# thallolang/thallo

Hardware: AMD Instinct MI355X
Metric: pcg_iters_per_sec (higher is better)
Workload: dtype f32

## Files before the change

thallo_amd/csrc/energy_image_warping_march_rc.hip:

```cpp
#include "iw_march.hpp"
#include <hip/hip_ext.h>

using namespace thallo;

namespace {

inline int check_launch() { hipError_t e = hipGetLastError(); return e == hipSuccess ? 0 : -(int)e; }

typedef __amdgpu_buffer_rsrc_t rsrc_t;
typedef unsigned u32x4 __attribute__((ext_vector_type(4)));
typedef unsigned u32x2 __attribute__((ext_vector_type(2)));
__device__ __forceinline__ rsrc_t make_rsrc(const void* p) { return __builtin_amdgcn_make_buffer_rsrc(const_cast<void*>(p), 0, 0xffffffffu, 0x00020000); }
template <bool NT> __device__ __forceinline__ u32x4 bld4(rsrc_t r, unsigned vo, unsigned so) { return __builtin_amdgcn_raw_buffer_load_b128(r, vo, so, NT ? 2 : 0); }
template <bool NT> __device__ __forceinline__ u32x2 bld2(rsrc_t r, unsigned vo, unsigned so) { return __builtin_amdgcn_raw_buffer_load_b64(r, vo, so, NT ? 2 : 0); }
template <bool NT> __device__ __forceinline__ unsigned bld1(rsrc_t r, unsigned vo, unsigned so) { return __builtin_amdgcn_raw_buffer_load_b32(r, vo, so, NT ? 2 : 0); }
template <bool NT> __device__ __forceinline__ void bst4(rsrc_t r, unsigned vo, unsigned so, float a, float b, float c, float d)
{ u32x4 v; v.x = __float_as_uint(a); v.y = __float_as_uint(b); v.z = __float_as_uint(c); v.w = __float_as_uint(d); __builtin_amdgcn_raw_buffer_store_b128(v, r, vo, so, NT ? 2 : 0); }
template <bool NT> __device__ __forceinline__ void bst2(rsrc_t r, unsigned vo, unsigned so, float a, float b)
{ u32x2 v; v.x = __float_as_uint(a); v.y = __float_as_uint(b); __builtin_amdgcn_raw_buffer_store_b64(v, r, vo, so, NT ? 2 : 0); }
__device__ __forceinline__ float uf(unsigned u) { return __uint_as_float(u); }
__device__ __forceinline__ float to_sgpr(float v) { return __int_as_float(__builtin_amdgcn_readfirstlane(__float_as_int(v))); }

__device__ __forceinline__ float rc_sum(thallo_sum_t s)
{
    if (s.count == 1) return s.partials[0];
    float t = 0.0f;
    for (int i = threadIdx.x & (THALLO_WAVE - 1); i < s.count; i += THALLO_WAVE) t += s.partials[i];
    return wave_sum_all(t);
}
__device__ __forceinline__ void rc_iteration_scalars(thallo_sum_t aNp, thallo_sum_t aDp, thallo_sum_t bNp, const PrevSums& prev, float& alpha, float& beta, bool writer)
{
    const float an = rc_sum(aNp);
    float ad, bn;
    if (prev.count > 0) {
        const int lane = threadIdx.x & (THALLO_WAVE - 1), nb = prev.count;
        float t = 0.0f; double n = 0.0, a1 = 0.0, b1 = 0.0;
        for (int i = lane; i < nb; i += THALLO_WAVE) { t += prev.aD_part[i]; n += prev.s12_part[3 * i]; a1 += prev.s12_part[3 * i + 1]; b1 += prev.s12_part[3 * i + 2]; }
        ad = nb == 1 ? prev.aD_part[0] : wave_sum_all(t);
        n = wave_sum_all_d(n); a1 = wave_sum_all_d(a1); b1 = wave_sum_all_d(b1);
        alpha = safe_div<false>(an, ad);
        double bd = n - 2.0 * (double)alpha * a1 + (double)alpha * (double)alpha * b1;
        if (!(bd > 0.0)) bd = 0.0;
        bn = (float)bd;
        if (writer) { prev.aD_word[0] = ad; prev.bN_word[0] = bn; }
    } else {
        ad = rc_sum(aDp); bn = rc_sum(bNp);
        alpha = safe_div<false>(an, ad);
    }
    beta = safe_div<false>(bn, an);
}

__device__ __forceinline__ void rc_exchange_prev(thallo_sum_t aNp, const PrevSums& prev, const thallo_dist_t& dd)
{
    typedef unsigned long long u64_t;
    const unsigned seq = ld_agent(dd.ctl + DIST_SEQ);
    const unsigned tag = (seq << 12) | (unsigned)(prev.xslot / 7 + 1);
    const IterationSums S = load_iteration_sums(prev.aD_part, prev.s12_part, prev.count, aNp);
    float ad = 0.0f, al = 0.0f, bn = 0.0f;
    dist_exchange_iter_wave_seq(dd, seq, prev.xslot, S.ad, S.n, S.s1, S.s2, S.an, prev.aD_word, prev.bN_word, ExtraSums{ false, 0.0f, 0.0, 0.0, 0.0 }, &ad, &al, &bn);
    if ((threadIdx.x & (THALLO_WAVE - 1)) == 0) {
        __hip_atomic_store(prev.gs, ((u64_t)tag << 32) | (u64_t)__float_as_uint(ad), __ATOMIC_RELAXED, __HIP_MEMORY_SCOPE_AGENT);
        __hip_atomic_store(prev.gs + 1, ((u64_t)tag << 32) | (u64_t)__float_as_uint(bn), __ATOMIC_RELAXED, __HIP_MEMORY_SCOPE_AGENT);
    }
}
__device__ __forceinline__ void rc_iteration_scalars_x(thallo_sum_t aNp, const PrevSums& prev, const thallo_dist_t& dd, float& alpha, float& beta)
{
    typedef unsigned long long u64_t;
    const float an = rc_sum(aNp);
    const unsigned seq = ld_agent(dd.ctl + DIST_SEQ);
    const unsigned tag = (seq << 12) | (unsigned)(prev.xslot / 7 + 1);
    u64_t v0 = __hip_atomic_load(prev.gs, __ATOMIC_RELAXED, __HIP_MEMORY_SCOPE_AGENT), v1 = __hip_atomic_load(prev.gs + 1, __ATOMIC_RELAXED, __HIP_MEMORY_SCOPE_AGENT);
    int it = 0; long long t0 = 0;
    const long long bound = dist_spin_ticks(dd);
    while ((unsigned)(v0 >> 32) != tag || (unsigned)(v1 >> 32) != tag) {
        if ((it & 255) == 0) { if (ld_agent(dd.ctl + DIST_ERR) != 0) break; if (it == 0) t0 = wall_clock64(); }
        ++it;
        if ((it & 255) == 0 && wall_clock64() - t0 > bound) {
            if (__hip_atomic_exchange(dd.ctl + DIST_ERR, 1u, __ATOMIC_RELAXED, __HIP_MEMORY_SCOPE_AGENT) == 0u) {
                unsigned* pm = dd.ctl + DIST_POST_MORTEM;
                pm[0] = (unsigned)prev.xslot; pm[1] = 0xffffu; pm[2] = tag; pm[3] = (unsigned)(v0 >> 32); pm[4] = (unsigned)(v1 >> 32);
            }
            break;
        }
        __builtin_amdgcn_s_sleep(4);
        v0 = __hip_atomic_load(prev.gs, __ATOMIC_RELAXED, __HIP_MEMORY_SCOPE_AGENT); v1 = __hip_atomic_load(prev.gs + 1, __ATOMIC_RELAXED, __HIP_MEMORY_SCOPE_AGENT);
    }
    const float ad = __uint_as_float((unsigned)v0), bn = __uint_as_float((unsigned)v1);
    alpha = safe_div<false>(an, ad);
    beta = safe_div<false>(bn, an);
}
__global__ __launch_bounds__(64) void k_rc_dist_finish(thallo_sum_t aNp, PrevSums prev, thallo_dist_t dd) { rc_exchange_prev(aNp, prev, dd); }

template <int DMODE>
struct RawRc {
    u32x4 po, cs; u32x2 pa; unsigned f;
    u32x4 ro; u32x2 ra;
    u32x4 dlo, ppo; u32x2 dla, ppa;
};
typedef unsigned long long u64x2 __attribute__((ext_vector_type(2)));
__device__ __forceinline__ void take4u(u32x4& d, const u32x4& s) { const u64x2 sv = __builtin_bit_cast(u64x2, s); unsigned long long a, b; take_pair(a, sv.x); take_pair(b, sv.y); u64x2 dv; dv.x = a; dv.y = b; d = __builtin_bit_cast(u32x4, dv); }
__device__ __forceinline__ void take2u(u32x2& d, const u32x2& s) { unsigned long long a; take_pair(a, __builtin_bit_cast(unsigned long long, s)); d = __builtin_bit_cast(u32x2, a); }
template <int DMODE>
__device__ __forceinline__ void take(RawRc<DMODE>& d, const RawRc<DMODE>& s)
{
    take4u(d.po, s.po); take2u(d.pa, s.pa); take4u(d.cs, s.cs); take1(d.f, s.f); take4u(d.ro, s.ro); take2u(d.ra, s.ra);
    if (DMODE != 1) { take4u(d.dlo, s.dlo); take2u(d.dla, s.dla); }
    if (DMODE == 2) { take4u(d.ppo, s.ppo); take2u(d.ppa, s.ppa); }
}

struct PRow { v2f xy[2]; float pa[2]; };
struct GRow { v2f cs[2], gx[2]; float a[2]; unsigned f; };
struct RRow { v2f xy[2]; float ra[2]; };
__device__ __forceinline__ v2f uf2(unsigned a, unsigned b) { return v2f{ uf(a), uf(b) }; }

template <int DMODE, int DEPTH, int NTM, int OCC, int SLAB>
__global__ __launch_bounds__(MARCH_NT, OCC) void k_iter_march_rc(MarchGeo g, const float* __restrict__ cs, const unsigned char* __restrict__ flags, float wf2, float wr2,
                                                            const float* __restrict__ r_in, float* __restrict__ r_out, const float* __restrict__ A_in, float* __restrict__ A_out,
                                                            const float* __restrict__ p_in, float* __restrict__ p_out, float* __restrict__ delta,
                                                            thallo_sum_t aNp, thallo_sum_t aDp, thallo_sum_t bNp, thallo_sum_t aNpp, thallo_sum_t aDpp,
                                                            float* __restrict__ aD_out, double* __restrict__ s12_out, const int* __restrict__ irregular,
                                                            thallo_dist_t dd, unsigned* __restrict__ fin_tickets, float* __restrict__ aD_word, float* __restrict__ bN_word, int xslot,
                                                            PrevSums prev)
{
    static_assert(DEPTH == 1 || DEPTH == 2 || DEPTH == 4, "the prefetch slots rotate inside a trip of four rows");
    __shared__ float4 lut[32];
    __shared__ float red[16];
    __shared__ double redd[48];
    constexpr bool nt_delta = NTM & 1, nt_ra = NTM & 2, nt_out = NTM & 4, nt_pin = NTM & 8, nt_pout = NTM & 16, nt_const = NTM & 32;
    if (irregular != nullptr && __builtin_amdgcn_readfirstlane(irregular[0]) != 0) {
        if (blockIdx.x == 0 && threadIdx.x == 0 && aD_word) { aD_word[0] = __builtin_nanf(""); bN_word[0] = __builtin_nanf(""); }
        if (blockIdx.x == 0 && threadIdx.x == 0 && prev.count > 0) { prev.aD_word[0] = __builtin_nanf(""); prev.bN_word[0] = __builtin_nanf(""); }
        if (threadIdx.x == 0) { aD_out[blockIdx.x] = __builtin_nanf(""); }
        return;
    }
    if (threadIdx.x < 32) { float mo, ma; pre_from_flags((unsigned char)threadIdx.x, wf2, wr2, mo, ma); lut[threadIdx.x] = make_float4(mo, ma, (threadIdx.x & 2) ? wf2 : 0.f, 0.f); }
    __syncthreads();

    const int lane = threadIdx.x & 63, wave = __builtin_amdgcn_readfirstlane(threadIdx.x >> 6);
    const unsigned N = (unsigned)g.W * (unsigned)g.H;
    const int W2 = g.W >> 1;
    int strip, ya, yb;
    march_place(g, wave, strip, ya, yb);
    const bool work = ya < yb;
    const int x0 = strip * MARCH_USE - 2 + 2 * lane;
    const bool xin = x0 >= 0 && x0 < g.W;
    const bool xout = xin && lane >= 1 && lane <= 62;

    const rsrc_t RS_P = make_rsrc(p_in), RS_R = make_rsrc(r_in), RS_CS = make_rsrc(cs), RS_F = make_rsrc(flags);
    const rsrc_t RS_Q = make_rsrc(p_out), RS_RO = make_rsrc(r_out), RS_D = make_rsrc(delta);
    const rsrc_t RS_AI = make_rsrc(SLAB ? (const void*)A_in : (const void*)r_in), RS_AO = make_rsrc(SLAB ? (void*)A_out : (void*)r_out);
    const int xc = x0 < 0 ? 0 : x0 > g.W - 2 ? g.W - 2 : x0;
    const unsigned h = (unsigned)xc >> 1;
    const unsigned vo16 = h * 16u, vo8 = h * 8u;
    const unsigned vf0 = (h >> 1) * 4u, vf1 = ((h + 1u) >> 1) * 4u, sh0 = (h & 1u) * 16u;
    const unsigned angle0 = 8u * N;

    float alpha = 0.0f, beta = 0.0f, alpha2 = 0.0f;
    const bool scal_writer = work && strip == 0 && ya == g.row0 && lane == 0;

    typedef RawRc<DMODE> RawT;
    RawT slot[DEPTH];
    auto issue = [&](RawT& s, int t) {
        const unsigned tc = (unsigned)(t < 0 ? 0 : t > g.H - 1 ? g.H - 1 : t), row = tc * (unsigned)W2;
        s.po = bld4<nt_pin>(RS_P, vo16, row * 16u); s.pa = bld2<nt_pin>(RS_P, vo8, angle0 + row * 8u);
        s.cs = bld4<nt_const>(RS_CS, vo16, row * 16u);
        const unsigned par = row & 1u;
        s.f = bld1<nt_const>(RS_F, par ? vf1 : vf0, (row - par) * 2u);
        const unsigned tr = (unsigned)(t - 1 < 0 ? 0 : t - 1 > g.H - 1 ? g.H - 1 : t - 1), rrow = tr * (unsigned)W2;
        s.ro = bld4<nt_ra>(RS_R, vo16, rrow * 16u); s.ra = bld2<nt_ra>(RS_R, vo8, angle0 + rrow * 8u);
        if (DMODE != 1) {
            const unsigned td = (unsigned)(t - 1 < ya ? ya : t - 1 > yb - 1 ? yb - 1 : t - 1), drow = td * (unsigned)W2;
            s.dlo = bld4<nt_delta>(RS_D, vo16, drow * 16u); s.dla = bld2<nt_delta>(RS_D, vo8, angle0 + drow * 8u);
            if (DMODE == 2) { s.ppo = bld4<false>(RS_Q, vo16, drow * 16u); s.ppa = bld2<false>(RS_Q, vo8, angle0 + drow * 8u); }
        }
    };

    PRow pp[4], pk[4]; GRow gg[4]; RRow rr[2];
#pragma unroll
    for (int i = 0; i < 4; ++i) {
#pragma unroll
        for (int q = 0; q < 2; ++q) { pp[i].xy[q] = v2f{ 0.f, 0.f }; pp[i].pa[q] = 0.f; pk[i].xy[q] = v2f{ 0.f, 0.f }; pk[i].pa[q] = 0.f;
                                      gg[i].cs[q] = v2f{ 1.f, 0.f }; gg[i].gx[q] = v2f{ 0.f, -1.f }; gg[i].a[q] = 0.f; }
        gg[i].f = 0u;
    }
#pragma unroll
    for (int i = 0; i < 2; ++i)
#pragma unroll
        for (int q = 0; q < 2; ++q) { rr[i].xy[q] = v2f{ 0.f, 0.f }; rr[i].ra[q] = 0.f; }

    float acc = 0.0f; double s0 = 0.0, s1 = 0.0, s2 = 0.0;
    const unsigned mxin = xin ? 0xffffu : 0u;
    if (SLAB == 2 && prev.gs != nullptr && prev.count > 0 && blockIdx.x == gridDim.x - 1 && wave == 0 && !work) rc_exchange_prev(aNp, prev, dd);

    if (work) {
        const int t_first = ya - 2, t_last = yb + 1;
#pragma unroll
        for (int j = 0; j < DEPTH; ++j) slot[j] = RawT{};
        const int t_begin = t_first - DEPTH;
        for (int t0 = t_begin; t0 <= t_last; t0 += 4) {
            if (DEPTH == 1 ? t0 == t_begin : t0 == t_begin + 4) {
                if (SLAB == 2 && prev.gs != nullptr && prev.count > 0) rc_iteration_scalars_x(aNp, prev, dd, alpha, beta);
                else rc_iteration_scalars(aNp, aDp, bNp, prev, alpha, beta, scal_writer);
                alpha = to_sgpr(alpha); beta = to_sgpr(beta);
                if (DMODE == 2) alpha2 = to_sgpr(safe_div<false>(rc_sum(aNpp), rc_sum(aDpp)));
            }
#pragma unroll
            for (int j = 0; j < 4; ++j) {
                const int t = t0 + j;
                PRow& p0 = pp[j % 4]; const PRow& p1 = pp[(j + 3) % 4]; const PRow& p2 = pp[(j + 2) % 4];
                GRow& g0 = gg[j % 4]; const GRow& g1 = gg[(j + 3) % 4]; const GRow& g2 = gg[(j + 2) % 4]; const GRow& g3 = gg[(j + 1) % 4];
                PRow& k1 = pk[(j + 3) % 4]; const PRow& k2 = pk[(j + 2) % 4]; const PRow& k3 = pk[(j + 1) % 4];
                RRow& r1 = rr[(j + 1) % 2]; const RRow& r2 = rr[j % 2];
                RawT cur;
                take(cur, slot[j % DEPTH]);
                fence_order();
                issue(slot[j % DEPTH], t + DEPTH > t_last ? t_last : t + DEPTH);
                fence_order();
                {
                    const bool rowok = t >= 0 && t < g.H;
                    const unsigned par = ((unsigned)t * (unsigned)W2) & 1u;
                    const unsigned fl = (cur.f >> (par ? 16u - sh0 : sh0)) & (rowok ? mxin : 0u);
                    p0.xy[0] = uf2(cur.po.x, cur.po.y); p0.xy[1] = uf2(cur.po.z, cur.po.w); p0.pa[0] = uf(cur.pa.x); p0.pa[1] = uf(cur.pa.y);
                    g0.cs[0] = uf2(cur.cs.x, cur.cs.y); g0.cs[1] = uf2(cur.cs.z, cur.cs.w); g0.f = fl;
                    g0.gx[0] = v2f{ g0.cs[0].y, -g0.cs[0].x }; g0.gx[1] = v2f{ g0.cs[1].y, -g0.cs[1].x };
                    g0.a[0] = (float)(fl & 1u); g0.a[1] = (float)((fl >> 8) & 1u);
                }
                const int u = t - 1;
                {
                    const float4 m0 = lut[g1.f & 31u], m1 = lut[(g1.f >> 8) & 31u];
                    const float wfit[2] = { m0.z, m1.z };
                    v2f axy[2]; float av[2];
                    jtjp_pair_xy(p2, p1, p0, g2, g1, g0, g2.a, g1.a, g0.a, wfit, wr2, axy, av);
                    const bool ghost_row = SLAB && ((u == ya - 1 && ya == g.row0 && u >= 0) || (u == yb && yb == g.row1 && u < g.H));
                    if (ghost_row) {
                        const unsigned row = (unsigned)u * (unsigned)W2;
                        const u32x4 ao = bld4<false>(RS_AI, vo16, row * 16u); const u32x2 aa = bld2<false>(RS_AI, vo8, angle0 + row * 8u);
                        axy[0] = uf2(ao.x, ao.y); axy[1] = uf2(ao.z, ao.w); av[0] = uf(aa.x); av[1] = uf(aa.y);
                    }
                    v2f rxy[2] = { uf2(cur.ro.x, cur.ro.y), uf2(cur.ro.z, cur.ro.w) }; float rq[2] = { uf(cur.ra.x), uf(cur.ra.y) };
                    rxy[0] = fma2(-alpha, axy[0], rxy[0]); rxy[1] = fma2(-alpha, axy[1], rxy[1]);
                    rq[0] = __builtin_fmaf(-alpha, av[0], rq[0]); rq[1] = __builtin_fmaf(-alpha, av[1], rq[1]);
                    const float mo[2] = { m0.x, m1.x }, ma[2] = { m0.y, m1.y };
#pragma unroll
                    for (int q = 0; q < 2; ++q) {
                        k1.xy[q] = mo[q] * rxy[q] + beta * p1.xy[q]; k1.pa[q] = ma[q] * rq[q] + beta * p1.pa[q];
                        r1.xy[q] = rxy[q]; r1.ra[q] = rq[q];
                    }
                    const bool mine = u >= ya && u < yb;
                    if (xout && (mine || ghost_row)) {
                        const unsigned row = (unsigned)u * (unsigned)W2;
                        bst4<nt_out>(RS_RO, vo16, row * 16u, rxy[0].x, rxy[0].y, rxy[1].x, rxy[1].y); bst2<nt_out>(RS_RO, vo8, angle0 + row * 8u, rq[0], rq[1]);
                        bst4<nt_pout>(RS_Q, vo16, row * 16u, k1.xy[0].x, k1.xy[0].y, k1.xy[1].x, k1.xy[1].y); bst2<nt_pout>(RS_Q, vo8, angle0 + row * 8u, k1.pa[0], k1.pa[1]);
                        if (DMODE != 1 && mine) {
                            float d[4] = { uf(cur.dlo.x), uf(cur.dlo.y), uf(cur.dlo.z), uf(cur.dlo.w) }, da[2] = { uf(cur.dla.x), uf(cur.dla.y) };
                            if (DMODE == 2) {
                                d[0] = __builtin_fmaf(alpha2, uf(cur.ppo.x), d[0]); d[1] = __builtin_fmaf(alpha2, uf(cur.ppo.y), d[1]);
                                d[2] = __builtin_fmaf(alpha2, uf(cur.ppo.z), d[2]); d[3] = __builtin_fmaf(alpha2, uf(cur.ppo.w), d[3]);
                                da[0] = __builtin_fmaf(alpha2, uf(cur.ppa.x), da[0]); da[1] = __builtin_fmaf(alpha2, uf(cur.ppa.y), da[1]);
                            }
                            d[0] = __builtin_fmaf(alpha, p1.xy[0].x, d[0]); d[1] = __builtin_fmaf(alpha, p1.xy[0].y, d[1]);
                            d[2] = __builtin_fmaf(alpha, p1.xy[1].x, d[2]); d[3] = __builtin_fmaf(alpha, p1.xy[1].y, d[3]);
                            da[0] = __builtin_fmaf(alpha, p1.pa[0], da[0]); da[1] = __builtin_fmaf(alpha, p1.pa[1], da[1]);
                            bst4<nt_delta>(RS_D, vo16, row * 16u, d[0], d[1], d[2], d[3]); bst2<nt_delta>(RS_D, vo8, angle0 + row * 8u, da[0], da[1]);
                        }
                    }
                }
                __builtin_amdgcn_sched_barrier(0);
                {
                    const int v = t - 2;
                    const bool on = xout && v >= ya && v < yb;
                    const float4 m0 = lut[on ? g2.f & 31u : 0u], m1 = lut[on ? (g2.f >> 8) & 31u : 0u];
                    const float wfit[2] = { m0.z, m1.z }, mo[2] = { m0.x, m1.x }, ma[2] = { m0.y, m1.y };
                    v2f axy[2]; float av[2];
                    jtjp_pair_xy(k3, k2, k1, g3, g2, g1, g3.a, g2.a, g1.a, wfit, wr2, axy, av);
                    if (SLAB && xout && v >= ya && v < yb && (v == g.row0 || v == g.row1 - 1)) {
                        if (SLAB == 1) {
                            const unsigned row = (unsigned)v * (unsigned)W2;
                            bst4<false>(RS_AO, vo16, row * 16u, axy[0].x, axy[0].y, axy[1].x, axy[1].y); bst2<false>(RS_AO, vo8, angle0 + row * 8u, av[0], av[1]);
                        } else {
#pragma unroll
                            for (int k = 0; k < 2; ++k) {
                                if (v == (k == 0 ? g.row0 : g.row1 - 1) && dd.peer_r[k]) {
                                    float* d2 = dd.peer_r[k] + dd.peer_off_o[k] + 2 * x0;
                                    st_sys(d2, axy[0].x); st_sys(d2 + 1, axy[0].y); st_sys(d2 + 2, axy[1].x); st_sys(d2 + 3, axy[1].y);
                                    float* d1 = dd.peer_r[k] + dd.peer_off_a[k] + x0;
                                    st_sys(d1, av[0]); st_sys(d1 + 1, av[1]);
                                }
                            }
                        }
                    }
                    const float msum = on ? 1.0f : 0.0f;
                    __builtin_amdgcn_sched_barrier(0);
                    iter_sums_pixel_masked(msum, k2.xy[0].x, k2.xy[0].y, k2.pa[0], axy[0].x, axy[0].y, av[0], r2.xy[0].x, r2.xy[0].y, r2.ra[0], mo[0], ma[0], acc, s0, s1, s2);
                    __builtin_amdgcn_sched_barrier(0);
                    iter_sums_pixel_masked(msum, k2.xy[1].x, k2.xy[1].y, k2.pa[1], axy[1].x, axy[1].y, av[1], r2.xy[1].x, r2.xy[1].y, r2.ra[1], mo[1], ma[1], acc, s0, s1, s2);
                }
                asm volatile("" : "+v"(acc), "+v"(s0), "+v"(s1), "+v"(s2));
                __builtin_amdgcn_sched_barrier(0);
            }
        }
    }
    iter_tail<MARCH_NT, SLAB == 2>(acc, s0, s1, s2, red, redd, aD_out, s12_out, bNp, &dd, fin_tickets, aD_word, bN_word, xslot);
}

}

[[maybe_unused]] constexpr int MARCH_RC_DEPTH = 4;
constexpr int MARCH_RC_OCC = 2;
[[maybe_unused]] constexpr int MARCH_RC_DEEP_ROWS = 24;
#ifdef THALLO_MARCH_SWEEP
namespace thallo {
int g_march_rc_depth = MARCH_RC_DEPTH;
int g_march_rc_occ = MARCH_RC_OCC;
int g_march_rc_nt = MARCH_NTM;
}
#endif

namespace {
struct LaunchEvents { hipEvent_t start = nullptr, stop = nullptr; int armed = 0, used = 0; };
thread_local LaunchEvents g_launch_ev;

template <int SLAB>
int launch_march_rc(int W, int H, int row0, int row1, const float* cs, const unsigned char* flags, float w_fit, float w_reg,
                    const float* r_in, float* r_out, const float* A_in, float* A_out, const float* p_in, float* p_out, float* delta, int mode,
                    thallo_sum_t aNp, thallo_sum_t aDp, thallo_sum_t bNp, thallo_sum_t aNpp, thallo_sum_t aDpp, const int* irregular, thallo_dist_t d,
                    float* aD_out, double* s12_out, unsigned* fin_tickets, float* aD_word, float* bN_word, int xslot, hipStream_t stream, PrevSums prev)
{
    const int R = march_pick_rows(W, row1 - row0);
    if (R <= 0) return -(int)hipErrorNotSupported;
    const MarchGeo g = make_march_geo(W, H, row0, row1, R);
    const int grid = (g.total + 7) / 8 * 8 + ((SLAB == 2 && prev.gs != nullptr) ? 8 : 0);
    if (grid > THALLO_MAX_PARTIALS) return -(int)hipErrorInvalidValue;
    const int dmode = (mode >> 1) & 3;
    const float wf2 = w_fit * w_fit, wr2 = w_reg * w_reg;
    const bool ev_on = g_launch_ev.armed != 0;
    if (ev_on) g_launch_ev.used = 1;
#define RC_LAUNCH(DM, DP, OCC, NTM) do { if (ev_on) hipExtLaunchKernelGGL((k_iter_march_rc<DM, DP, NTM, OCC, SLAB>), dim3(grid), dim3(MARCH_NT), 0, stream, g_launch_ev.start, g_launch_ev.stop, 0, g, cs, flags, wf2, wr2, \
        r_in, r_out, A_in, A_out, p_in, p_out, delta, aNp, aDp, bNp, aNpp, aDpp, aD_out, s12_out, irregular, d, fin_tickets, aD_word, bN_word, xslot, prev); \
    else hipLaunchKernelGGL((k_iter_march_rc<DM, DP, NTM, OCC, SLAB>), dim3(grid), dim3(MARCH_NT), 0, stream, g, cs, flags, wf2, wr2, \
        r_in, r_out, A_in, A_out, p_in, p_out, delta, aNp, aDp, bNp, aNpp, aDpp, aD_out, s12_out, irregular, d, fin_tickets, aD_word, bN_word, xslot, prev); } while (0)
#ifdef THALLO_MARCH_SWEEP
#define RC_BY_DEPTH(DM) do { if constexpr (SLAB != 0) RC_LAUNCH(DM, MARCH_RC_DEPTH, MARCH_RC_OCC, MARCH_NTM); else { const int dp = g_march_rc_depth, oc = g_march_rc_occ, nt = g_march_rc_nt; \
        if (nt != MARCH_NTM) { if (nt == 0) RC_LAUNCH(DM, MARCH_RC_DEPTH, 2, 0); else if (nt == 1) RC_LAUNCH(DM, MARCH_RC_DEPTH, 2, 1); else if (nt == 4) RC_LAUNCH(DM, MARCH_RC_DEPTH, 2, 4); else if (nt == 7) RC_LAUNCH(DM, MARCH_RC_DEPTH, 2, 7); \
                                 else if (nt == 13) RC_LAUNCH(DM, MARCH_RC_DEPTH, 2, 13); else if (nt == 21) RC_LAUNCH(DM, MARCH_RC_DEPTH, 2, 21); else if (nt == 37) RC_LAUNCH(DM, MARCH_RC_DEPTH, 2, 37); else if (nt == 63) RC_LAUNCH(DM, MARCH_RC_DEPTH, 2, 63); else return -(int)hipErrorInvalidValue; } \
        else if (oc == 1) { if (dp == 4) RC_LAUNCH(DM, 4, 1, MARCH_NTM); else RC_LAUNCH(DM, 2, 1, MARCH_NTM); } \
        else if (oc == 3) { if (dp == 1) RC_LAUNCH(DM, 1, 3, MARCH_NTM); else RC_LAUNCH(DM, 2, 3, MARCH_NTM); } \
        else { if (dp == 1) RC_LAUNCH(DM, 1, 2, MARCH_NTM); else if (dp == 4) RC_LAUNCH(DM, 4, 2, MARCH_NTM); else RC_LAUNCH(DM, 2, 2, MARCH_NTM); } } } while (0)
#else
#define RC_BY_DEPTH(DM) do { if (R >= MARCH_RC_DEEP_ROWS) RC_LAUNCH(DM, 4, MARCH_RC_OCC, MARCH_NTM); else RC_LAUNCH(DM, 2, MARCH_RC_OCC, MARCH_NTM); } while (0)
#endif
    if (dmode == 1) RC_BY_DEPTH(1); else if (dmode == 2) RC_BY_DEPTH(2); else RC_BY_DEPTH(0);
#undef RC_BY_DEPTH
#undef RC_LAUNCH
    int e = check_launch(); return e ? e : grid;
}

int rc_check(int W, int H, int row0, int row1, const void* cs, const void* flags, const void* r_in, const void* r_out, const void* A_in, const void* A_out,
             const void* p_in, const void* p_out, const void* delta, int mode, thallo_sum_t aNp, thallo_sum_t aNpp, thallo_sum_t aDpp, const void* aD_out, const void* s12_out)
{
    if ((W & 1) || W < 2 || H < 1 || row0 < 0 || row1 > H || row0 >= row1 || row0 > 1 || H - row1 > 1) return -(int)hipErrorInvalidValue;
    if (mode & 1) return -(int)hipErrorInvalidValue;
    if (!cs || !flags || !r_in || !r_out || !p_in || !p_out || !delta || !aD_out || !s12_out) return -(int)hipErrorInvalidValue;
    if ((row0 > 0 || row1 < H) && (!A_in || !A_out)) return -(int)hipErrorInvalidValue;
    if (aNp.count < 1 || !aNp.partials) return -(int)hipErrorInvalidValue;
    if (((mode >> 1) & 3) == 2 && (aNpp.count < 1 || aDpp.count < 1 || !aNpp.partials || !aDpp.partials)) return -(int)hipErrorInvalidValue;
    if (12.0 * (double)W * (double)H >= 4294967296.0) return -(int)hipErrorNotSupported;
    return 0;
}
}

extern "C" {

int thallo_hip_iw_pcg_iter_march_rc(int W, int H, int row0, int row1, const float* cs, const unsigned char* flags, float w_fit, float w_reg,
                                    const float* r_in, float* r_out, const float* Ap_in, float* Ap_out, const float* p_in, float* p_out, float* delta, int mode,
                                    thallo_sum_t aNp, thallo_sum_t aDp, thallo_sum_t bNp, thallo_sum_t aNpp, thallo_sum_t aDpp,
                                    const int* irregular, float* aD_out, double* s12_out,
                                    unsigned* fin_tickets, float* aD_word, float* bN_word, thallo_stream_t stream)
{
    if (int e = rc_check(W, H, row0, row1, cs, flags, r_in, r_out, Ap_in, Ap_out, p_in, p_out, delta, mode, aNp, aNpp, aDpp, aD_out, s12_out)) return e;
    if (aDp.count < 1 || bNp.count < 1 || !aDp.partials || !bNp.partials) return -(int)hipErrorInvalidValue;
    if (!fin_tickets || !aD_word || !bN_word) { fin_tickets = nullptr; aD_word = nullptr; bN_word = nullptr; }
    const PrevSums none = { nullptr, nullptr, 0, nullptr, nullptr };
    if (row0 == 0 && row1 == H)
        return launch_march_rc<0>(W, H, row0, row1, cs, flags, w_fit, w_reg, r_in, r_out, nullptr, nullptr, p_in, p_out, delta, mode, aNp, aDp, bNp, aNpp, aDpp, irregular, thallo_dist_t{},
                                  aD_out, s12_out, fin_tickets, aD_word, bN_word, 0, (hipStream_t)stream, none);
    return launch_march_rc<1>(W, H, row0, row1, cs, flags, w_fit, w_reg, r_in, r_out, Ap_in, Ap_out, p_in, p_out, delta, mode, aNp, aDp, bNp, aNpp, aDpp, irregular, thallo_dist_t{},
                              aD_out, s12_out, fin_tickets, aD_word, bN_word, 0, (hipStream_t)stream, none);
}

int thallo_hip_iw_pcg_iter_march_rc_deferred(int W, int H, int row0, int row1, const float* cs, const unsigned char* flags, float w_fit, float w_reg,
                                             const float* r_in, float* r_out, const float* Ap_in, float* Ap_out, const float* p_in, float* p_out, float* delta, int mode,
                                             thallo_sum_t aNp, thallo_sum_t aNpp, thallo_sum_t aDpp, thallo_prev_t prev,
                                             const int* irregular, float* aD_out, double* s12_out, thallo_stream_t stream)
{
    if (int e = rc_check(W, H, row0, row1, cs, flags, r_in, r_out, Ap_in, Ap_out, p_in, p_out, delta, mode, aNp, aNpp, aDpp, aD_out, s12_out)) return e;
    if (prev.count < 1 || prev.count > THALLO_MAX_PARTIALS || !prev.alphaD_partials || !prev.s12_partials || !prev.alphaD_word || !prev.betaN_word ||
        prev.s12_partials == s12_out) return -(int)hipErrorInvalidValue;
    const thallo_sum_t none = { nullptr, 0 };
    const PrevSums ps = { prev.alphaD_partials, prev.s12_partials, prev.count, prev.alphaD_word, prev.betaN_word };
    if (row0 == 0 && row1 == H)
        return launch_march_rc<0>(W, H, row0, row1, cs, flags, w_fit, w_reg, r_in, r_out, nullptr, nullptr, p_in, p_out, delta, mode, aNp, none, none, aNpp, aDpp, irregular, thallo_dist_t{},
                                  aD_out, s12_out, nullptr, nullptr, nullptr, 0, (hipStream_t)stream, ps);
    return launch_march_rc<1>(W, H, row0, row1, cs, flags, w_fit, w_reg, r_in, r_out, Ap_in, Ap_out, p_in, p_out, delta, mode, aNp, none, none, aNpp, aDpp, irregular, thallo_dist_t{},
                              aD_out, s12_out, nullptr, nullptr, nullptr, 0, (hipStream_t)stream, ps);
}

int thallo_hip_iw_pcg_iter_march_rc_dist(int W, int H, int row0, int row1, const float* cs, const unsigned char* flags, float w_fit, float w_reg,
                                         const float* r_in, float* r_out, const float* Ap_in, float* Ap_out, const float* p_in, float* p_out, float* delta, int mode,
                                         thallo_sum_t aNp, thallo_sum_t aDp, thallo_sum_t bNp, thallo_sum_t aNpp, thallo_sum_t aDpp,
                                         const int* irregular, thallo_dist_t d, float* aD_out, double* s12_out,
                                         unsigned* fin_tickets, int slot0, float* aD_word, float* bN_word, thallo_stream_t stream)
{
    if (int e = rc_check(W, H, row0, row1, cs, flags, r_in, r_out, Ap_in, Ap_out, p_in, p_out, delta, mode, aNp, aNpp, aDpp, aD_out, s12_out)) return e;
    if (!Ap_in || !Ap_out || aDp.count < 1 || bNp.count < 1 || !aDp.partials || !bNp.partials || d.world < 1 || d.world > THALLO_DIST_MAX_WORLD) return -(int)hipErrorInvalidValue;
    if (!fin_tickets || !aD_word || !bN_word) { fin_tickets = nullptr; aD_word = nullptr; bN_word = nullptr; }
    if (fin_tickets && (slot0 < 0 || !d.mail || !d.ctl || 7 * d.world > 64 || bNp.count != 1)) return -(int)hipErrorInvalidValue;
    for (int k = 0; k < 2; ++k) if (d.peer_r[k] && ((d.peer_off_o[k] | d.peer_off_a[k]) & 1)) return -(int)hipErrorInvalidValue;
    return launch_march_rc<2>(W, H, row0, row1, cs, flags, w_fit, w_reg, r_in, r_out, Ap_in, Ap_out, p_in, p_out, delta, mode, aNp, aDp, bNp, aNpp, aDpp, irregular, d,
                              aD_out, s12_out, fin_tickets, aD_word, bN_word, slot0, (hipStream_t)stream, PrevSums{ nullptr, nullptr, 0, nullptr, nullptr });
}

int thallo_hip_iw_march_rc_deferred_fits(int W, int rows)
{
    if (W < 2 || (W & 1) || rows < 1) return 0;
    const int R = march_pick_rows(W, rows);
    if (R <= 0) return 0;
    const MarchGeo g = make_march_geo(W, rows, 0, rows, R);
    const long grid = (g.total + 7) / 8 * 8 + 8;
    return grid <= march_cap(MARCH_RC_OCC) && grid <= THALLO_MAX_PARTIALS ? 1 : 0;
}

int thallo_hip_iw_pcg_iter_march_rc_dist_deferred(int W, int H, int row0, int row1, const float* cs, const unsigned char* flags, float w_fit, float w_reg,
                                                  const float* r_in, float* r_out, const float* Ap_in, float* Ap_out, const float* p_in, float* p_out, float* delta, int mode,
                                                  thallo_sum_t aNp, thallo_sum_t aNpp, thallo_sum_t aDpp, thallo_prev_t prev, int prev_slot0, unsigned long long* gs,
                                                  const int* irregular, thallo_dist_t d, float* aD_out, double* s12_out, thallo_stream_t stream)
{
    if (int e = rc_check(W, H, row0, row1, cs, flags, r_in, r_out, Ap_in, Ap_out, p_in, p_out, delta, mode, aNp, aNpp, aDpp, aD_out, s12_out)) return e;
    if (!Ap_in || !Ap_out || d.world < 1 || d.world > THALLO_DIST_MAX_WORLD || !d.mail || !d.ctl || 7 * d.world > 64 || prev_slot0 < 0 || !gs || aNp.count != 1) return -(int)hipErrorInvalidValue;
    if (!thallo_hip_iw_march_rc_deferred_fits(W, row1 - row0)) return -(int)hipErrorNotSupported;
    if (prev.count < 1 || prev.count > THALLO_MAX_PARTIALS || !prev.alphaD_partials || !prev.s12_partials || !prev.alphaD_word || !prev.betaN_word ||
        prev.s12_partials == s12_out) return -(int)hipErrorInvalidValue;
    for (int k = 0; k < 2; ++k) if (d.peer_r[k] && ((d.peer_off_o[k] | d.peer_off_a[k]) & 1)) return -(int)hipErrorInvalidValue;
    const thallo_sum_t none = { nullptr, 0 };
    const PrevSums ps = { prev.alphaD_partials, prev.s12_partials, prev.count, prev.alphaD_word, prev.betaN_word, gs, prev_slot0 };
    return launch_march_rc<2>(W, H, row0, row1, cs, flags, w_fit, w_reg, r_in, r_out, Ap_in, Ap_out, p_in, p_out, delta, mode, aNp, none, none, aNpp, aDpp, irregular, d,
                              aD_out, s12_out, nullptr, nullptr, nullptr, 0, (hipStream_t)stream, ps);
}
int thallo_hip_iw_dist_finish_deferred(thallo_prev_t prev, int prev_slot0, thallo_sum_t aNp, thallo_dist_t d, unsigned long long* gs, thallo_stream_t stream)
{
    if (prev.count < 1 || prev.count > THALLO_MAX_PARTIALS || !prev.alphaD_partials || !prev.s12_partials || !prev.alphaD_word || !prev.betaN_word || prev_slot0 < 0 || !gs ||
        aNp.count != 1 || !aNp.partials || d.world < 1 || d.world > THALLO_DIST_MAX_WORLD || !d.mail || !d.ctl || 7 * d.world > 64) return -(int)hipErrorInvalidValue;
    const PrevSums ps = { prev.alphaD_partials, prev.s12_partials, prev.count, prev.alphaD_word, prev.betaN_word, gs, prev_slot0 };
    hipLaunchKernelGGL(k_rc_dist_finish, dim3(1), dim3(64), 0, (hipStream_t)stream, aNp, ps, d);
    return check_launch();
}

void thallo_hip_march_rc_debug_set(int what, int value)
{
#ifdef THALLO_MARCH_SWEEP
    if (what == 0) g_march_rc_depth = value;
    if (what == 1) g_march_rc_occ = value;
    if (what == 2) g_march_rc_nt = value;
#else
    (void)what; (void)value;
#endif
}

void thallo_hip_launch_events_arm(void* start, void* stop) { g_launch_ev.start = (hipEvent_t)start; g_launch_ev.stop = (hipEvent_t)stop; g_launch_ev.armed = start && stop ? 1 : 0; g_launch_ev.used = 0; }
int thallo_hip_launch_events_take(void) { const int u = g_launch_ev.used; g_launch_ev = LaunchEvents(); return u; }

}
```

Measured before the change: 16290.

## Peel march loop into prologue, unclamped steady state and clamped tail phases

Restructures the row-marching loop into compile-time phases. The warm-up rows skip the JtJ computations that cannot yet be valid, and the steady-state body runs without per-row clamping or bounds checks on row indices and ownership masks. A clamped tail handles the last rows. This is meant to cut scalar and vector overhead from index clamps and predicates in the hot loop, at the cost of larger code and a risk of subtle edge bugs in the boundary logic.

```diff
diff --git a/thallo_amd/csrc/energy_image_warping_march_rc.hip b/thallo_amd/csrc/energy_image_warping_march_rc.hip
--- a/thallo_amd/csrc/energy_image_warping_march_rc.hip
+++ b/thallo_amd/csrc/energy_image_warping_march_rc.hip
@@ -108,6 +108,9 @@
     if (DMODE == 2) { take4u(d.ppo, s.ppo); take2u(d.ppa, s.ppa); }
 }
 
+template <int V> struct IC { static constexpr int value = V; };
+enum { PH_ENTER = 0, PH_S1 = 1, PH_FULL = 2 };
+
 struct PRow { v2f xy[2]; float pa[2]; };
 struct GRow { v2f cs[2], gx[2]; float a[2]; unsigned f; };
 struct RRow { v2f xy[2]; float ra[2]; };
@@ -160,16 +163,20 @@
 
     typedef RawRc<DMODE> RawT;
     RawT slot[DEPTH];
-    auto issue = [&](RawT& s, int t) {
-        const unsigned tc = (unsigned)(t < 0 ? 0 : t > g.H - 1 ? g.H - 1 : t), row = tc * (unsigned)W2;
+    const unsigned W2u = (unsigned)W2;
+    const int t_first = ya - 2, t_last = yb + 1;
+    auto issue = [&](RawT& s, int tn, auto CL_) __attribute__((always_inline)) {
+        constexpr bool CL = decltype(CL_)::value;
+        if (CL && tn > t_last) tn = t_last;
+        const unsigned tc = CL ? (unsigned)(tn < 0 ? 0 : tn > g.H - 1 ? g.H - 1 : tn) : (unsigned)tn, row = tc * W2u;
         s.po = bld4<nt_pin>(RS_P, vo16, row * 16u); s.pa = bld2<nt_pin>(RS_P, vo8, angle0 + row * 8u);
         s.cs = bld4<nt_const>(RS_CS, vo16, row * 16u);
         const unsigned par = row & 1u;
         s.f = bld1<nt_const>(RS_F, par ? vf1 : vf0, (row - par) * 2u);
-        const unsigned tr = (unsigned)(t - 1 < 0 ? 0 : t - 1 > g.H - 1 ? g.H - 1 : t - 1), rrow = tr * (unsigned)W2;
+        const unsigned tr = CL ? (unsigned)(tn - 1 < 0 ? 0 : tn - 1 > g.H - 1 ? g.H - 1 : tn - 1) : (unsigned)(tn - 1), rrow = tr * W2u;
         s.ro = bld4<nt_ra>(RS_R, vo16, rrow * 16u); s.ra = bld2<nt_ra>(RS_R, vo8, angle0 + rrow * 8u);
         if (DMODE != 1) {
-            const unsigned td = (unsigned)(t - 1 < ya ? ya : t - 1 > yb - 1 ? yb - 1 : t - 1), drow = td * (unsigned)W2;
+            const unsigned td = CL ? (unsigned)(tn - 1 < ya ? ya : tn - 1 > yb - 1 ? yb - 1 : tn - 1) : (unsigned)(tn - 1), drow = td * W2u;
             s.dlo = bld4<nt_delta>(RS_D, vo16, drow * 16u); s.dla = bld2<nt_delta>(RS_D, vo8, angle0 + drow * 8u);
             if (DMODE == 2) { s.ppo = bld4<false>(RS_Q, vo16, drow * 16u); s.ppa = bld2<false>(RS_Q, vo8, angle0 + drow * 8u); }
         }
@@ -190,115 +197,130 @@
 
     float acc = 0.0f; double s0 = 0.0, s1 = 0.0, s2 = 0.0;
     const unsigned mxin = xin ? 0xffffu : 0u;
-    if (SLAB == 2 && prev.gs != nullptr && prev.count > 0 && blockIdx.x == gridDim.x - 1 && wave == 0 && !work) rc_exchange_prev(aNp, prev, dd);
-
-    if (work) {
-        const int t_first = ya - 2, t_last = yb + 1;
-#pragma unroll
-        for (int j = 0; j < DEPTH; ++j) slot[j] = RawT{};
-        const int t_begin = t_first - DEPTH;
-        for (int t0 = t_begin; t0 <= t_last; t0 += 4) {
-            if (DEPTH == 1 ? t0 == t_begin : t0 == t_begin + 4) {
-                if (SLAB == 2 && prev.gs != nullptr && prev.count > 0) rc_iteration_scalars_x(aNp, prev, dd, alpha, beta);
-                else rc_iteration_scalars(aNp, aDp, bNp, prev, alpha, beta, scal_writer);
-                alpha = to_sgpr(alpha); beta = to_sgpr(beta);
-                if (DMODE == 2) alpha2 = to_sgpr(safe_div<false>(rc_sum(aNpp), rc_sum(aDpp)));
+
+    auto step = [&](int t, auto J_, auto PH_, auto CL_) __attribute__((always_inline)) {
+        constexpr int j = decltype(J_)::value, PH = decltype(PH_)::value;
+        constexpr bool CL = decltype(CL_)::value;
+        PRow& p0 = pp[j % 4]; const PRow& p1 = pp[(j + 3) % 4]; const PRow& p2 = pp[(j + 2) % 4];
+        GRow& g0 = gg[j % 4]; const GRow& g1 = gg[(j + 3) % 4]; const GRow& g2 = gg[(j + 2) % 4]; const GRow& g3 = gg[(j + 1) % 4];
+        PRow& k1 = pk[(j + 3) % 4]; const PRow& k2 = pk[(j + 2) % 4]; const PRow& k3 = pk[(j + 1) % 4];
+        RRow& r1 = rr[(j + 1) % 2]; const RRow& r2 = rr[j % 2];
+        RawT cur;
+        take(cur, slot[j % DEPTH]);
+        fence_order();
+        issue(slot[j % DEPTH], t + DEPTH, CL_);
+        fence_order();
+        {
+            const bool rowok = !CL || (t >= 0 && t < g.H);
+            const unsigned par = ((unsigned)t * W2u) & 1u;
+            const unsigned fl = (cur.f >> (par ? 16u - sh0 : sh0)) & (rowok ? mxin : 0u);
+            p0.xy[0] = uf2(cur.po.x, cur.po.y); p0.xy[1] = uf2(cur.po.z, cur.po.w); p0.pa[0] = uf(cur.pa.x); p0.pa[1] = uf(cur.pa.y);
+            g0.cs[0] = uf2(cur.cs.x, cur.cs.y); g0.cs[1] = uf2(cur.cs.z, cur.cs.w); g0.f = fl;
+            g0.gx[0] = v2f{ g0.cs[0].y, -g0.cs[0].x }; g0.gx[1] = v2f{ g0.cs[1].y, -g0.cs[1].x };
+            g0.a[0] = (float)(fl & 1u); g0.a[1] = (float)((fl >> 8) & 1u);
+        }
+        if constexpr (PH >= PH_S1) {
+            const int u = t - 1;
+            const float4 m0 = lut[g1.f & 31u], m1 = lut[(g1.f >> 8) & 31u];
+            const float wfit[2] = { m0.z, m1.z };
+            v2f axy[2]; float av[2];
+            jtjp_pair_xy(p2, p1, p0, g2, g1, g0, g2.a, g1.a, g0.a, wfit, wr2, axy, av);
+            const bool ghost_row = SLAB && CL && ((u == ya - 1 && ya == g.row0 && u >= 0) || (u == yb && yb == g.row1 && u < g.H));
+            if (ghost_row) {
+                const unsigned row = (unsigned)u * W2u;
+                const u32x4 ao = bld4<false>(RS_AI, vo16, row * 16u); const u32x2 aa = bld2<false>(RS_AI, vo8, angle0 + row * 8u);
+                axy[0] = uf2(ao.x, ao.y); axy[1] = uf2(ao.z, ao.w); av[0] = uf(aa.x); av[1] = uf(aa.y);
             }
-#pragma unroll
-            for (int j = 0; j < 4; ++j) {
-                const int t = t0 + j;
-                PRow& p0 = pp[j % 4]; const PRow& p1 = pp[(j + 3) % 4]; const PRow& p2 = pp[(j + 2) % 4];
-                GRow& g0 = gg[j % 4]; const GRow& g1 = gg[(j + 3) % 4]; const GRow& g2 = gg[(j + 2) % 4]; const GRow& g3 = gg[(j + 1) % 4];
-                PRow& k1 = pk[(j + 3) % 4]; const PRow& k2 = pk[(j + 2) % 4]; const PRow& k3 = pk[(j + 1) % 4];
-                RRow& r1 = rr[(j + 1) % 2]; const RRow& r2 = rr[j % 2];
-                RawT cur;
-                take(cur, slot[j % DEPTH]);
-                fence_order();
-                issue(slot[j % DEPTH], t + DEPTH > t_last ? t_last : t + DEPTH);
-                fence_order();
-                {
-                    const bool rowok = t >= 0 && t < g.H;
-                    const unsigned par = ((unsigned)t * (unsigned)W2) & 1u;
-                    const unsigned fl = (cur.f >> (par ? 16u - sh0 : sh0)) & (rowok ? mxin : 0u);
-                    p0.xy[0] = uf2(cur.po.x, cur.po.y); p0.xy[1] = uf2(cur.po.z, cur.po.w); p0.pa[0] = uf(cur.pa.x); p0.pa[1] = uf(cur.pa.y);
-                    g0.cs[0] = uf2(cur.cs.x, cur.cs.y); g0.cs[1] = uf2(cur.cs.z, cur.cs.w); g0.f = fl;
-                    g0.gx[0] = v2f{ g0.cs[0].y, -g0.cs[0].x }; g0.gx[1] = v2f{ g0.cs[1].y, -g0.cs[1].x };
-                    g0.a[0] = (float)(fl & 1u); g0.a[1] = (float)((fl >> 8) & 1u);
+            v2f rxy[2] = { uf2(cur.ro.x, cur.ro.y), uf2(cur.ro.z, cur.ro.w) }; float rq[2] = { uf(cur.ra.x), uf(cur.ra.y) };
+            rxy[0] = fma2(-alpha, axy[0], rxy[0]); rxy[1] = fma2(-alpha, axy[1], rxy[1]);
+            rq[0] = __builtin_fmaf(-alpha, av[0], rq[0]); rq[1] = __builtin_fmaf(-alpha, av[1], rq[1]);
+            const float mo[2] = { m0.x, m1.x }, ma[2] = { m0.y, m1.y };
+#pragma unroll
+            for (int q = 0; q < 2; ++q) {
+                k1.xy[q] = mo[q] * rxy[q] + beta * p1.xy[q]; k1.pa[q] = ma[q] * rq[q] + beta * p1.pa[q];
+                r1.xy[q] = rxy[q]; r1.ra[q] = rq[q];
+            }
+            const bool mine = !CL || (u >= ya && u < yb);
+            if (xout && (mine || ghost_row)) {
+                const unsigned row = (unsigned)u * W2u;
+                bst4<nt_out>(RS_RO, vo16, row * 16u, rxy[0].x, rxy[0].y, rxy[1].x, rxy[1].y); bst2<nt_out>(RS_RO, vo8, angle0 + row * 8u, rq[0], rq[1]);
+                bst4<nt_pout>(RS_Q, vo16, row * 16u, k1.xy[0].x, k1.xy[0].y, k1.xy[1].x, k1.xy[1].y); bst2<nt_pout>(RS_Q, vo8, angle0 + row * 8u, k1.pa[0], k1.pa[1]);
+                if (DMODE != 1 && mine) {
+                    float d[4] = { uf(cur.dlo.x), uf(cur.dlo.y), uf(cur.dlo.z), uf(cur.dlo.w) }, da[2] = { uf(cur.dla.x), uf(cur.dla.y) };
+                    if (DMODE == 2) {
+                        d[0] = __builtin_fmaf(alpha2, uf(cur.ppo.x), d[0]); d[1] = __builtin_fmaf(alpha2, uf(cur.ppo.y), d[1]);
+                        d[2] = __builtin_fmaf(alpha2, uf(cur.ppo.z), d[2]); d[3] = __builtin_fmaf(alpha2, uf(cur.ppo.w), d[3]);
+                        da[0] = __builtin_fmaf(alpha2, uf(cur.ppa.x), da[0]); da[1] = __builtin_fmaf(alpha2, uf(cur.ppa.y), da[1]);
+                    }
+                    d[0] = __builtin_fmaf(alpha, p1.xy[0].x, d[0]); d[1] = __builtin_fmaf(alpha, p1.xy[0].y, d[1]);
+                    d[2] = __builtin_fmaf(alpha, p1.xy[1].x, d[2]); d[3] = __builtin_fmaf(alpha, p1.xy[1].y, d[3]);
+                    da[0] = __builtin_fmaf(alpha, p1.pa[0], da[0]); da[1] = __builtin_fmaf(alpha, p1.pa[1], da[1]);
+                    bst4<nt_delta>(RS_D, vo16, row * 16u, d[0], d[1], d[2], d[3]); bst2<nt_delta>(RS_D, vo8, angle0 + row * 8u, da[0], da[1]);
                 }
-                const int u = t - 1;
-                {
-                    const float4 m0 = lut[g1.f & 31u], m1 = lut[(g1.f >> 8) & 31u];
-                    const float wfit[2] = { m0.z, m1.z };
-                    v2f axy[2]; float av[2];
-                    jtjp_pair_xy(p2, p1, p0, g2, g1, g0, g2.a, g1.a, g0.a, wfit, wr2, axy, av);
-                    const bool ghost_row = SLAB && ((u == ya - 1 && ya == g.row0 && u >= 0) || (u == yb && yb == g.row1 && u < g.H));
-                    if (ghost_row) {
-                        const unsigned row = (unsigned)u * (unsigned)W2;
-                        const u32x4 ao = bld4<false>(RS_AI, vo16, row * 16u); const u32x2 aa = bld2<false>(RS_AI, vo8, angle0 + row * 8u);
-                        axy[0] = uf2(ao.x, ao.y); axy[1] = uf2(ao.z, ao.w); av[0] = uf(aa.x); av[1] = uf(aa.y);
-                    }
-                    v2f rxy[2] = { uf2(cur.ro.x, cur.ro.y), uf2(cur.ro.z, cur.ro.w) }; float rq[2] = { uf(cur.ra.x), uf(cur.ra.y) };
-                    rxy[0] = fma2(-alpha, axy[0], rxy[0]); rxy[1] = fma2(-alpha, axy[1], rxy[1]);
-                    rq[0] = __builtin_fmaf(-alpha, av[0], rq[0]); rq[1] = __builtin_fmaf(-alpha, av[1], rq[1]);
-                    const float mo[2] = { m0.x, m1.x }, ma[2] = { m0.y, m1.y };
-#pragma unroll
-                    for (int q = 0; q < 2; ++q) {
-                        k1.xy[q] = mo[q] * rxy[q] + beta * p1.xy[q]; k1.pa[q] = ma[q] * rq[q] + beta * p1.pa[q];
-                        r1.xy[q] = rxy[q]; r1.ra[q] = rq[q];
-                    }
-                    const bool mine = u >= ya && u < yb;
-                    if (xout && (mine || ghost_row)) {
-                        const unsigned row = (unsigned)u * (unsigned)W2;
-                        bst4<nt_out>(RS_RO, vo16, row * 16u, rxy[0].x, rxy[0].y, rxy[1].x, rxy[1].y); bst2<nt_out>(RS_RO, vo8, angle0 + row * 8u, rq[0], rq[1]);
-                        bst4<nt_pout>(RS_Q, vo16, row * 16u, k1.xy[0].x, k1.xy[0].y, k1.xy[1].x, k1.xy[1].y); bst2<nt_pout>(RS_Q, vo8, angle0 + row * 8u, k1.pa[0], k1.pa[1]);
-                        if (DMODE != 1 && mine) {
-                            float d[4] = { uf(cur.dlo.x), uf(cur.dlo.y), uf(cur.dlo.z), uf(cur.dlo.w) }, da[2] = { uf(cur.dla.x), uf(cur.dla.y) };
-                            if (DMODE == 2) {
-                                d[0] = __builtin_fmaf(alpha2, uf(cur.ppo.x), d[0]); d[1] = __builtin_fmaf(alpha2, uf(cur.ppo.y), d[1]);
-                                d[2] = __builtin_fmaf(alpha2, uf(cur.ppo.z), d[2]); d[3] = __builtin_fmaf(alpha2, uf(cur.ppo.w), d[3]);
-                                da[0] = __builtin_fmaf(alpha2, uf(cur.ppa.x), da[0]); da[1] = __builtin_fmaf(alpha2, uf(cur.ppa.y), da[1]);
-                            }
-                            d[0] = __builtin_fmaf(alpha, p1.xy[0].x, d[0]); d[1] = __builtin_fmaf(alpha, p1.xy[0].y, d[1]);
-                            d[2] = __builtin_fmaf(alpha, p1.xy[1].x, d[2]); d[3] = __builtin_fmaf(alpha, p1.xy[1].y, d[3]);
-                            da[0] = __builtin_fmaf(alpha, p1.pa[0], da[0]); da[1] = __builtin_fmaf(alpha, p1.pa[1], da[1]);
-                            bst4<nt_delta>(RS_D, vo16, row * 16u, d[0], d[1], d[2], d[3]); bst2<nt_delta>(RS_D, vo8, angle0 + row * 8u, da[0], da[1]);
+            }
+        }
+        __builtin_amdgcn_sched_barrier(0);
+        if constexpr (PH >= PH_FULL) {
+            const int v = t - 2;
+            const bool on = xout;
+            const float4 m0 = lut[on ? g2.f & 31u : 0u], m1 = lut[on ? (g2.f >> 8) & 31u : 0u];
+            const float wfit[2] = { m0.z, m1.z }, mo[2] = { m0.x, m1.x }, ma[2] = { m0.y, m1.y };
+            v2f axy[2]; float av[2];
+            jtjp_pair_xy(k3, k2, k1, g3, g2, g1, g3.a, g2.a, g1.a, wfit, wr2, axy, av);
+            if (SLAB && xout && (v == g.row0 || v == g.row1 - 1)) {
+                if (SLAB == 1) {
+                    const unsigned row = (unsigned)v * W2u;
+                    bst4<false>(RS_AO, vo16, row * 16u, axy[0].x, axy[0].y, axy[1].x, axy[1].y); bst2<false>(RS_AO, vo8, angle0 + row * 8u, av[0], av[1]);
+                } else {
+#pragma unroll
+                    for (int k = 0; k < 2; ++k) {
+                        if (v == (k == 0 ? g.row0 : g.row1 - 1) && dd.peer_r[k]) {
+                            float* d2 = dd.peer_r[k] + dd.peer_off_o[k] + 2 * x0;
+                            st_sys(d2, axy[0].x); st_sys(d2 + 1, axy[0].y); st_sys(d2 + 2, axy[1].x); st_sys(d2 + 3, axy[1].y);
+                            float* d1 = dd.peer_r[k] + dd.peer_off_a[k] + x0;
+                            st_sys(d1, av[0]); st_sys(d1 + 1, av[1]);
                         }
                     }
                 }
-                __builtin_amdgcn_sched_barrier(0);
-                {
-                    const int v = t - 2;
-                    const bool on = xout && v >= ya && v < yb;
-                    const float4 m0 = lut[on ? g2.f & 31u : 0u], m1 = lut[on ? (g2.f >> 8) & 31u : 0u];
-                    const float wfit[2] = { m0.z, m1.z }, mo[2] = { m0.x, m1.x }, ma[2] = { m0.y, m1.y };
-                    v2f axy[2]; float av[2];
-                    jtjp_pair_xy(k3, k2, k1, g3, g2, g1, g3.a, g2.a, g1.a, wfit, wr2, axy, av);
-                    if (SLAB && xout && v >= ya && v < yb && (v == g.row0 || v == g.row1 - 1)) {
-                        if (SLAB == 1) {
-                            const unsigned row = (unsigned)v * (unsigned)W2;
-                            bst4<false>(RS_AO, vo16, row * 16u, axy[0].x, axy[0].y, axy[1].x, axy[1].y); bst2<false>(RS_AO, vo8, angle0 + row * 8u, av[0], av[1]);
-                        } else {
-#pragma unroll
-                            for (int k = 0; k < 2; ++k) {
-                                if (v == (k == 0 ? g.row0 : g.row1 - 1) && dd.peer_r[k]) {
-                                    float* d2 = dd.peer_r[k] + dd.peer_off_o[k] + 2 * x0;
-                                    st_sys(d2, axy[0].x); st_sys(d2 + 1, axy[0].y); st_sys(d2 + 2, axy[1].x); st_sys(d2 + 3, axy[1].y);
-                                    float* d1 = dd.peer_r[k] + dd.peer_off_a[k] + x0;
-                                    st_sys(d1, av[0]); st_sys(d1 + 1, av[1]);
-                                }
-                            }
-                        }
-                    }
-                    const float msum = on ? 1.0f : 0.0f;
-                    __builtin_amdgcn_sched_barrier(0);
-                    iter_sums_pixel_masked(msum, k2.xy[0].x, k2.xy[0].y, k2.pa[0], axy[0].x, axy[0].y, av[0], r2.xy[0].x, r2.xy[0].y, r2.ra[0], mo[0], ma[0], acc, s0, s1, s2);
-                    __builtin_amdgcn_sched_barrier(0);
-                    iter_sums_pixel_masked(msum, k2.xy[1].x, k2.xy[1].y, k2.pa[1], axy[1].x, axy[1].y, av[1], r2.xy[1].x, r2.xy[1].y, r2.ra[1], mo[1], ma[1], acc, s0, s1, s2);
-                }
-                asm volatile("" : "+v"(acc), "+v"(s0), "+v"(s1), "+v"(s2));
-                __builtin_amdgcn_sched_barrier(0);
             }
-        }
+            const float msum = on ? 1.0f : 0.0f;
+            __builtin_amdgcn_sched_barrier(0);
+            iter_sums_pixel_masked(msum, k2.xy[0].x, k2.xy[0].y, k2.pa[0], axy[0].x, axy[0].y, av[0], r2.xy[0].x, r2.xy[0].y, r2.ra[0], mo[0], ma[0], acc, s0, s1, s2);
+            __builtin_amdgcn_sched_barrier(0);
+            iter_sums_pixel_masked(msum, k2.xy[1].x, k2.xy[1].y, k2.pa[1], axy[1].x, axy[1].y, av[1], r2.xy[1].x, r2.xy[1].y, r2.ra[1], mo[1], ma[1], acc, s0, s1, s2);
+        }
+        asm volatile("" : "+v"(acc), "+v"(s0), "+v"(s1), "+v"(s2));
+        __builtin_amdgcn_sched_barrier(0);
+    };
+
+    if (SLAB == 2 && prev.gs != nullptr && prev.count > 0 && blockIdx.x == gridDim.x - 1 && wave == 0 && !work) rc_exchange_prev(aNp, prev, dd);
+
+    if (work) {
+#pragma unroll
+        for (int i = 0; i < DEPTH; ++i) issue(slot[i], t_first + i, IC<1>{});
+        step(t_first, IC<0>{}, IC<PH_ENTER>{}, IC<1>{});
+        step(t_first + 1, IC<1>{}, IC<PH_ENTER>{}, IC<1>{});
+        if (SLAB == 2 && prev.gs != nullptr && prev.count > 0) rc_iteration_scalars_x(aNp, prev, dd, alpha, beta);
+        else rc_iteration_scalars(aNp, aDp, bNp, prev, alpha, beta, scal_writer);
+        alpha = to_sgpr(alpha); beta = to_sgpr(beta);
+        if (DMODE == 2) alpha2 = to_sgpr(safe_div<false>(rc_sum(aNpp), rc_sum(aDpp)));
+        step(ya, IC<2>{}, IC<PH_S1>{}, IC<1>{});
+        step(ya + 1, IC<3>{}, IC<PH_S1>{}, IC<1>{});
+        int t_lim = t_last < g.H - 1 ? t_last : g.H - 1;
+        if (DMODE != 1 && yb < t_lim) t_lim = yb;
+        const int t_safe = t_lim - DEPTH;
+        int t = ya + 2;
+        for (; t + 3 <= t_safe; t += 4) {
+            step(t, IC<0>{}, IC<PH_FULL>{}, IC<0>{});
+            step(t + 1, IC<1>{}, IC<PH_FULL>{}, IC<0>{});
+            step(t + 2, IC<2>{}, IC<PH_FULL>{}, IC<0>{});
+            step(t + 3, IC<3>{}, IC<PH_FULL>{}, IC<0>{});
+        }
+        auto tail = [&](auto I_) __attribute__((always_inline)) {
+            constexpr int i = decltype(I_)::value;
+            if constexpr (i < DEPTH + 5) { if (t + i <= t_last) step(t + i, IC<i % 4>{}, IC<PH_FULL>{}, IC<1>{}); }
+        };
+        tail(IC<0>{}); tail(IC<1>{}); tail(IC<2>{}); tail(IC<3>{}); tail(IC<4>{}); tail(IC<5>{}); tail(IC<6>{}); tail(IC<7>{}); tail(IC<8>{});
     }
     iter_tail<MARCH_NT, SLAB == 2>(acc, s0, s1, s2, red, redd, aD_out, s12_out, bNp, &dd, fin_tickets, aD_word, bN_word, xslot);
 }
```

New measurement: 16880, median of 6. 1.04x the previous value.
